# wyhlovecpp/GPT-Image-Edit

Hardware: AMD Instinct MI355X
Metric: edited images/sec, 28-step FLUX-Kontext (VAE encode + 28 x MMDiT + VAE decode) (higher is better)
Workload: dtype bf16; 1 GPU; cfg2_single_512x512_28step; batch_per_gpu=1, global_batch=1, height=512, width=512, S_txt=512, S_tgt=1024, S_cond=1024, seq_len=2560, num_inference_steps=28, blocks=19 double + 38 single, parallelism=dp1

## Files before the change

### gpt_image_edit_amd/csrc/gemm_epilogue.h

```cpp
#pragma once

#include "mxfp8_quant.h"

constexpr int BM = 256;

struct TileRows {
  int ld, wrap, rpb, b0, r0;
  int rf;
  float inv;
  bool big;
  FK_DEV TileRows(const fk_rows& r, int m0, bool flat = false) {
    ld = (int)r.ld;
    if (flat) { rpb = 0x7fffffff; wrap = 0; b0 = 0; r0 = rf = m0; big = true; inv = 0.f; }
    else if (r.rows_per_batch <= 0) { rpb = 0x7fffffff; wrap = 0; b0 = 0; r0 = 0; rf = m0; big = true; inv = 0.f; }
    else {
      rpb = (int)(r.rows_per_batch > 0x7fffffff ? 0x7fffffff : r.rows_per_batch);
      b0 = (unsigned)m0 / (unsigned)rpb;
      r0 = rf = m0 - b0 * rpb;
      wrap = (int)(r.batch_stride - (int64_t)rpb * r.ld);
      big = rpb >= BM;
      inv = 1.0f / (float)rpb;
    }
  }
  FK_DEV int crossed(int ml) const {
    const int r = r0 + ml;
    const int one = r >= rpb ? 1 : 0;
    const int many = (int)(((float)r + 0.5f) * inv);
    return big ? one : many;
  }
  FK_DEV int off(int ml) const { return ml * ld + crossed(ml) * wrap; }
  FK_DEV int64_t first(const fk_rows& r) const {
    return (int64_t)b0 * r.batch_stride + (int64_t)rf * r.ld;
  }
};

template <int N>
FK_DEV float row_ror(float v) {
  return __int_as_float(__builtin_amdgcn_update_dpp(0, __float_as_int(v), 0x120 + N, 0xf, 0xf, false));
}
FK_DEV float row16_sum(float v) {
  v += row_ror<8>(v);
  v += row_ror<4>(v);
  v += row_ror<2>(v);
  v += row_ror<1>(v);
  return v;
}

FK_DEV int xcd_chunk_index() {
  const int nwg = gridDim.x;
  const int q = nwg >> 3, r = nwg & 7;
  const int xcd = blockIdx.x & 7, idx = blockIdx.x >> 3;
  return (xcd < r ? xcd * (q + 1) : r * (q + 1) + (xcd - r) * q) + idx;
}

template <bool M16>
struct FragMap {
  static FK_DEV int row(int lane, int q) { return M16 ? (q & 1) * 16 + (lane & 15) : (lane & 31); }
  static FK_DEV int col(int lane, int q) { return M16 ? (q >> 1) * 16 + (lane >> 4) * 4 : 8 * q + 4 * (lane >> 5); }
};
FK_DEV f32x4_t quad_get(const f32x16_t& v, int q) { return f32x4_t{v[4 * q], v[4 * q + 1], v[4 * q + 2], v[4 * q + 3]}; }
FK_DEV void quad_set(f32x16_t& v, int q, const f32x4_t& c) {
  v[4 * q] = c[0]; v[4 * q + 1] = c[1]; v[4 * q + 2] = c[2]; v[4 * q + 3] = c[3];
}

constexpr int WALK_CT_OFF = 65536;
FK_DEV void lds_barrier() { asm volatile("s_waitcnt lgkmcnt(0)\n\ts_barrier" ::: "memory"); }
template <int EPI, int BN, class C, int HALF = -1, int UB = 8, bool WALK = false>
FK_DEV void store_tile(const f32x16_t (&acc)[C::NF][C::MF], const fk_gemm_args& p, char* smem, int m0, int n0,
                       int wm, int wn, const u32x4_t* other = nullptr, int flat = 0, const u32x2_t (*bias_in)[4] = nullptr) {
  constexpr bool ADD_OTHER = HALF >= 0 && !WALK;
  constexpr int MF0 = HALF > 0 ? C::MF / 2 : 0, MF1 = HALF == 0 ? C::MF / 2 : C::MF;
  constexpr int row0 = HALF > 0 ? BM / 2 : 0;
  int tid = threadIdx.x;
  if constexpr (C::NTHREADS == 256 || WALK) asm volatile("" : "+v"(tid));
  const int lane = tid & 63;
  using FM = FragMap<C::M16>;
  u32x2_t bw[C::NF][4];
#pragma unroll
  for (int nf = 0; nf < C::NF; ++nf)
#pragma unroll
    for (int q = 0; q < 4; ++q) bw[nf][q] = u32x2_t{0u, 0u};
  if constexpr (WALK) {
#pragma unroll
    for (int nf = 0; nf < C::NF; ++nf)
#pragma unroll
      for (int q = 0; q < 4; ++q) bw[nf][q] = bias_in[nf][q];
  } else if constexpr (EPI != FK_EPI_SCALE) {
    if (p.bias) {
#pragma unroll
      for (int nf = 0; nf < C::NF; ++nf)
#pragma unroll
        for (int q = 0; q < 4; ++q) {
          const int n = n0 + C::tile_col(wn, nf) + FM::col(lane, q);
          bw[nf][q] = *(const u32x2_t*)((const bf16_t*)p.bias + min(n, p.N - 4));
        }
    }
  }
  if constexpr (EPI == FK_EPI_F32DBG) {
#pragma unroll
    for (int nf = 0; nf < C::NF; ++nf)
#pragma unroll
      for (int q = 0; q < 4; ++q) {
        const int n = n0 + C::tile_col(wn, nf) + FM::col(lane, q);
        const float b[4] = {bf_lo(bw[nf][q][0]), bf_hi(bw[nf][q][0]), bf_lo(bw[nf][q][1]), bf_hi(bw[nf][q][1])};
#pragma unroll
        for (int mf = MF0; mf < MF1; ++mf) {
          const int m = m0 + C::tile_row(wm, mf) + FM::row(lane, q);
          f32x4_t x = quad_get(acc[nf][mf], q);
          if constexpr (HALF >= 0) {
#pragma unroll
            for (int j = 0; j < 4; ++j) x[j] += __uint_as_float(other[nf * 2 * C::MF + (mf - MF0) * 4 + q][j]);
          }
          if (m < p.M && n < p.N)
            *(f32x4_t*)((float*)p.C + fk_row_offset(p.c, m) + n) = f32x4_t{x[0] + b[0], x[1] + b[1], x[2] + b[2], x[3] + b[3]};
        }
      }
    return;
  }
  if constexpr (WALK) lds_barrier(); else __syncthreads();
  bf16_t* ct = WALK ? (bf16_t*)(smem + WALK_CT_OFF) - row0 * C::CT_LD : (bf16_t*)smem;
#pragma unroll
  for (int nf = 0; nf < C::NF; ++nf) {
#pragma unroll
    for (int q = 0; q < 4; ++q) {
      const int nl = C::tile_col(wn, nf) + FM::col(lane, q);
      const float b[4] = {bf_lo(bw[nf][q][0]), bf_hi(bw[nf][q][0]), bf_lo(bw[nf][q][1]), bf_hi(bw[nf][q][1])};
#pragma unroll
      for (int mf = MF0; mf < MF1; ++mf) {
        float v[4];
#pragma unroll
        for (int j = 0; j < 4; ++j) {
          float x = acc[nf][mf][q * 4 + j];
          if constexpr (ADD_OTHER) x += __uint_as_float(other[nf * 2 * C::MF + (mf - MF0) * 4 + q][j]);
          if constexpr (EPI == FK_EPI_SCALE) v[j] = x * p.alpha;
          else v[j] = x + b[j];
        }
        if constexpr (EPI == FK_EPI_GELU_TANH || EPI == FK_EPI_SILU) {
          round_bf_pair(v[0], v[1]);
          round_bf_pair(v[2], v[3]);
#pragma unroll
          for (int j = 0; j < 4; ++j) v[j] = EPI == FK_EPI_GELU_TANH ? gelu_tanh_f(v[j]) : silu_f(v[j]);
        }
        u32x2_t pk;
        pk[0] = pack_bf2(v[0], v[1]);
        pk[1] = pack_bf2(v[2], v[3]);
        const int ml = C::tile_row(wm, mf) + FM::row(lane, q);
        *(u32x2_t*)(ct + ml * C::CT_LD + nl) = pk;
      }
    }
  }
  if constexpr (WALK) lds_barrier(); else __syncthreads();
  if constexpr (WALK && HALF <= 0) asm volatile("s_waitcnt vmcnt(0)" ::: "memory");
  constexpr int CPR = BN / 8;
  constexpr int ITERS = (HALF >= 0 ? BM / 2 : BM) * CPR / C::NTHREADS;
  constexpr int U = (EPI == FK_EPI_QKV && (ITERS > 8 || HALF >= 0)) ? 4 : UB;
  static_assert(ITERS % U == 0 && C::NTHREADS % CPR == 0, "epilogue batching");
  constexpr bool HAS_RES = EPI == FK_EPI_GATE_RES || EPI == FK_EPI_RES;
  const bool cflat = flat & 2, rflat = flat & 4, gflat = flat & 8;
  const TileRows crow(p.c, m0, cflat);
  bf16_t* const cbase = (bf16_t*)p.C + crow.first(p.c);
  const TileRows rrow = HAS_RES ? TileRows(p.r, m0, rflat) : crow;
  const bf16_t* const rbase = HAS_RES ? (const bf16_t*)p.res + rrow.first(p.r) : nullptr;
  fk_rows gr = {0, 0, 0};
  if constexpr (EPI == FK_EPI_GATE_RES) gr.rows_per_batch = p.gate_rows_per_batch;
  const TileRows grow(gr, m0, gflat);
  const int D = EPI == FK_EPI_QKV ? p.qkv_heads * 128 : 1;
  const int which = EPI == FK_EPI_QKV ? n0 / D : 0;
  const int cc = tid % CPR, ml0 = row0 + tid / CPR;
  constexpr int ML_STEP = C::NTHREADS / CPR;
  const int n = n0 + cc * 8;
  const int nc = min(n, p.N - 8);
  const int mlast = p.M - 1 - m0;

  if (EPI == FK_EPI_QKV && which < 2) {
    const int hn = n - which * D;
    const int head = hn >> 7, dch = hn & 127;
    const u32x4_t ww = *(const u32x4_t*)((const bf16_t*)(which == 0 ? p.wq : p.wk) + dch);
    bf16_t* const dst = (bf16_t*)(which == 0 ? p.q_out : p.k_out);
#pragma unroll
    for (int j0 = 0; j0 < ITERS; j0 += U) {
      u32x4_t y[U];
      f32x4_t t0[U], t1[U];
      int srow[U], bidx[U];
#pragma unroll
      for (int u = 0; u < U; ++u) {
        const int ml = ml0 + ML_STEP * (j0 + u);
        y[u] = *(const u32x4_t*)(ct + ml * C::CT_LD + cc * 8);
        const int mlc = min(ml, mlast);
        const int nb = crow.crossed(mlc);
        bidx[u] = crow.b0 + nb;
        srow[u] = p.qkv_s_offset + crow.r0 + mlc - nb * crow.rpb;
        const float* tp = p.rope_cs + (int64_t)srow[u] * 128 + dch;
        t0[u] = *(const f32x4_t*)tp;
        t1[u] = *(const f32x4_t*)(tp + 4);
      }
#pragma unroll
      for (int u = 0; u < U; ++u) {
        const int ml = ml0 + ML_STEP * (j0 + u);
        float xv[8];
        float ss = 0.f;
#pragma unroll
        for (int e = 0; e < 4; ++e) {
          xv[2 * e] = bf_lo(y[u][e]);
          xv[2 * e + 1] = bf_hi(y[u][e]);
          ss += xv[2 * e] * xv[2 * e] + xv[2 * e + 1] * xv[2 * e + 1];
        }
        ss = row16_sum(ss);
        const float rs = __builtin_amdgcn_rsqf(ss * (1.0f / 128) + 1e-6f);
        const float cs[4] = {t0[u][0], t0[u][2], t1[u][0], t1[u][2]};
        const float sn[4] = {t0[u][1], t0[u][3], t1[u][1], t1[u][3]};
        u32x4_t ow;
#pragma unroll
        for (int e = 0; e < 4; ++e) {
          float re = xv[2 * e] * rs, im = xv[2 * e + 1] * rs;
          round_bf_pair(re, im);
          re *= bf_lo(ww[e]);
          im *= bf_hi(ww[e]);
          round_bf_pair(re, im);
          const float o0 = mul2_add(re, cs[e], -im, sn[e]);
          const float o1 = mul2_add(im, cs[e], re, sn[e]);
          ow[e] = pack_bf2(o0, o1);
        }
        const int hrow = (bidx[u] * p.qkv_heads + head) * p.qkv_s_total + srow[u];
        if (ml <= mlast && n < p.N) *(u32x4_t*)(dst + (int64_t)hrow * 128 + dch) = ow;
      }
    }
    return;
  }

#pragma unroll
  for (int j0 = 0; j0 < ITERS; j0 += U) {
    u32x4_t y[U], rv[U], gv[U];
    int coff[U];
#pragma unroll
    for (int u = 0; u < U; ++u) {
      const int ml = ml0 + ML_STEP * (j0 + u);
      const int mlc = min(ml, mlast);
      y[u] = *(const u32x4_t*)(ct + ml * C::CT_LD + cc * 8);
      coff[u] = crow.off(mlc) + n;
      if constexpr (EPI == FK_EPI_GATE_RES || EPI == FK_EPI_RES) rv[u] = *(const u32x4_t*)(rbase + rrow.off(mlc) + nc);
      if constexpr (EPI == FK_EPI_GATE_RES) {
        const int64_t b = grow.b0 + grow.crossed(mlc);
        gv[u] = *(const u32x4_t*)((const bf16_t*)p.gate + b * p.gate_batch_stride + nc);
      }
    }
#pragma unroll
    for (int u = 0; u < U; ++u) {
      const int ml = ml0 + ML_STEP * (j0 + u);
      u32x4_t o = y[u];
      if constexpr (EPI == FK_EPI_GATE_RES || EPI == FK_EPI_RES) {
#pragma unroll
        for (int e = 0; e < 4; ++e) {
          float y0 = bf_lo(o[e]), y1 = bf_hi(o[e]);
          if constexpr (EPI == FK_EPI_GATE_RES) {
            y0 *= bf_lo(gv[u][e]);
            y1 *= bf_hi(gv[u][e]);
            round_bf_pair(y0, y1);
          }
          o[e] = pack_bf2(bf_lo(rv[u][e]) + y0, bf_hi(rv[u][e]) + y1);
        }
      }
      if (ml <= mlast && n < p.N) *(u32x4_t*)(cbase + coff[u]) = o;
    }
  }
}

template <int EPI, int BN, class C>
FK_DEV void store_tile_mxq(const f32x16_t (&acc)[C::NF][C::MF], const fk_gemm_args& p, uint8_t* __restrict__ q,
                           uint8_t* __restrict__ s, int64_t ldq, int64_t ld_scale, char* smem, int m0, int n0, int wm, int wn) {
  static_assert(EPI == FK_EPI_NONE || EPI == FK_EPI_GELU_TANH, "quantized output: plain and GELU epilogues");
  const int tid = threadIdx.x, lane = tid & 63;
  using FM = FragMap<C::M16>;
  u32x2_t bw[C::NF][4];
#pragma unroll
  for (int nf = 0; nf < C::NF; ++nf)
#pragma unroll
    for (int qd = 0; qd < 4; ++qd) bw[nf][qd] = u32x2_t{0u, 0u};
  if (p.bias) {
#pragma unroll
    for (int nf = 0; nf < C::NF; ++nf)
#pragma unroll
      for (int qd = 0; qd < 4; ++qd) {
        const int n = n0 + C::tile_col(wn, nf) + FM::col(lane, qd);
        bw[nf][qd] = *(const u32x2_t*)((const bf16_t*)p.bias + min(n, p.N - 4));
      }
  }
  __syncthreads();
  bf16_t* ct = (bf16_t*)smem;
#pragma unroll
  for (int nf = 0; nf < C::NF; ++nf) {
#pragma unroll
    for (int qd = 0; qd < 4; ++qd) {
      const int nl = C::tile_col(wn, nf) + FM::col(lane, qd);
      const float b[4] = {bf_lo(bw[nf][qd][0]), bf_hi(bw[nf][qd][0]), bf_lo(bw[nf][qd][1]), bf_hi(bw[nf][qd][1])};
#pragma unroll
      for (int mf = 0; mf < C::MF; ++mf) {
        float v[4];
#pragma unroll
        for (int j = 0; j < 4; ++j) v[j] = acc[nf][mf][qd * 4 + j] + b[j];
        if constexpr (EPI == FK_EPI_GELU_TANH) {
          round_bf_pair(v[0], v[1]);
          round_bf_pair(v[2], v[3]);
#pragma unroll
          for (int j = 0; j < 4; ++j) v[j] = gelu_tanh_f(v[j]);
        }
        u32x2_t pk;
        pk[0] = pack_bf2(v[0], v[1]);
        pk[1] = pack_bf2(v[2], v[3]);
        const int ml = C::tile_row(wm, mf) + FM::row(lane, qd);
        *(u32x2_t*)(ct + ml * C::CT_LD + nl) = pk;
      }
    }
  }
  __syncthreads();
  constexpr int BPR = BN / 32;
  constexpr int ITERS = BM * BPR / C::NTHREADS;
  constexpr int ML_STEP = C::NTHREADS / BPR;
  static_assert(C::NTHREADS % BPR == 0 && (BM * BPR) % C::NTHREADS == 0, "quantized epilogue tiling");
  const int bc = tid % BPR, ml0 = tid / BPR;
  const int mlast = p.M - 1 - m0;
#pragma unroll
  for (int j = 0; j < ITERS; ++j) {
    const int ml = ml0 + ML_STEP * j;
    const u32x4_t* src = (const u32x4_t*)(ct + ml * C::CT_LD + bc * 32);
    uint32_t w[16], out[8];
#pragma unroll
    for (int i = 0; i < 4; ++i) {
      const u32x4_t v = src[i];
      w[4 * i] = v[0]; w[4 * i + 1] = v[1]; w[4 * i + 2] = v[2]; w[4 * i + 3] = v[3];
    }
    const uint32_t sbyte = mx_quant_block(w, out);
    if (ml <= mlast) {
      const int64_t m = (int64_t)m0 + ml;
      u32x4_t* dst = (u32x4_t*)(q + m * ldq + n0 + bc * 32);
      dst[0] = u32x4_t{out[0], out[1], out[2], out[3]};
      dst[1] = u32x4_t{out[4], out[5], out[6], out[7]};
      s[m * ld_scale + (n0 >> 5) + bc] = (uint8_t)sbyte;
    }
  }
}
```

### gpt_image_edit_amd/csrc/gemm_pingpong_bf16.hip

```cpp
#include <stdlib.h>

#include <type_traits>

#include "fk_common.h"

namespace {

#include "gemm_epilogue.h"
#define FK_TM_FN __host__ __device__ __forceinline__
#include "gemm_tile_map.h"
static_assert(TM_MAX_GROUP == FK_MAX_GROUP && TM_BM == BM, "gemm_tile_map.h mirrors fk.h / gemm_epilogue.h");
#ifndef FK_GROUP_M
#define FK_GROUP_M 8
#endif
constexpr int GROUP_M = FK_GROUP_M;
#ifndef FK_RATE_256
#define FK_RATE_256 1.22
#endif


enum { SK_WHOLE = 0, SK_SYM = 1, SK_SYM_UNANNOUNCED = 2 };

struct GroupArgs {
  TileEntry e;
// ... 7 lines not shown
};


#ifdef FK_ENTRY_STAMPS
__device__ unsigned long long* fk_entry_stamp_buf = nullptr;
struct EntryStamps {
  unsigned long long t[5];
  template <int I> FK_DEV void mark() { t[I] = __builtin_amdgcn_s_memtime(); }
  FK_DEV void flush() const {
    if (threadIdx.x == 0 && fk_entry_stamp_buf) {
      unsigned long long* r = fk_entry_stamp_buf + (size_t)blockIdx.x * 8;
      for (int i = 0; i < 5; ++i) r[i] = t[i];
      r[5] = (unsigned long long)__builtin_amdgcn_s_getreg(63492) | ((unsigned long long)__builtin_amdgcn_s_getreg(63508) << 32);
    }
  }
};
#else
struct EntryStamps {
  template <int I> FK_DEV void mark() {}
  FK_DEV void flush() const {}
};
#endif

typedef __attribute__((address_space(3))) void lds_void;
typedef __attribute__((address_space(1))) const void gbl_void;

typedef short s16x4_t __attribute__((ext_vector_type(4)));
FK_DEV s16x4_t lds_tr16(const char* p) {
  return __builtin_amdgcn_ds_read_tr16_b64_v4i16((__attribute__((address_space(3))) s16x4_t*)p);
}

FK_DEV void buffer_lds16(__amdgpu_buffer_rsrc_t rsrc, char* lds_dst, int voffset, int soffset) {
#if defined(__HIP_DEVICE_COMPILE__)
  __builtin_amdgcn_raw_ptr_buffer_load_lds(rsrc, (lds_void*)lds_dst, 16, voffset, soffset, 0, 0);
#else
  (void)rsrc; (void)lds_dst; (void)voffset; (void)soffset;
#endif
}

FK_DEV void buffer_lds16(const BufDesc& d, char* lds_dst, int voffset, int soffset) {
  buffer_lds_opaque<16>(d, lds_addr_of(lds_dst), voffset, soffset);
}

template <int N>
FK_DEV void wait_vmcnt() {
  if constexpr (N == 0) asm volatile("s_waitcnt vmcnt(0)" ::: "memory");
  else if constexpr (N == 2) asm volatile("s_waitcnt vmcnt(2)" ::: "memory");
  else if constexpr (N == 4) asm volatile("s_waitcnt vmcnt(4)" ::: "memory");
  else if constexpr (N == 6) asm volatile("s_waitcnt vmcnt(6)" ::: "memory");
  else if constexpr (N == 8) asm volatile("s_waitcnt vmcnt(8)" ::: "memory");
  else if constexpr (N == 10) asm volatile("s_waitcnt vmcnt(10)" ::: "memory");
  else if constexpr (N == 12) asm volatile("s_waitcnt vmcnt(12)" ::: "memory");
  else if constexpr (N == 7) asm volatile("s_waitcnt vmcnt(7)" ::: "memory");
  else static_assert(N == 0, "add the vmcnt literal");
}


struct Hot {
  TmHot h;
  uint32_t xq, xr, grid;
  int nk;
};
#define FK_PIN_CLASS(h)                                                                                                   \
  "+s"((h).before[0]), "+s"((h).before[1]), "+s"((h).before[2]), "+s"((h).nbm[0]), "+s"((h).nbm[1]), "+s"((h).nbm[2]),       \
      "+s"((h).nbm[3]), "+s"((h).last_mul[0]), "+s"((h).last_mul[1]), "+s"((h).last_mul[2]), "+s"((h).last_mul[3]),          \
      "+s"((h).per_group), "+s"((h).col0), "+s"((h).per_group_mul), "+s"((h).group_m_mul)
#define FK_PIN_HEAD(x) "+s"((x).h.n), "+s"((x).h.group_m), "+s"((x).xq), "+s"((x).xr), "+s"((x).grid), "+s"((x).nk)
FK_DEV Hot load_hot(const GroupArgs& ga) {
  Hot x;
  x.h = tm_hot(ga.e, ga.e.cls[0]);
  x.xq = ga.e.xq; x.xr = ga.e.xr; x.grid = ga.e.grid; x.nk = ga.e.nk;
  asm volatile("" : FK_PIN_HEAD(x), FK_PIN_CLASS(x.h));
  return x;
}
FK_DEV ProbEntry load_prob(const GroupArgs& ga, int pi) {
  ProbEntry q = ga.pe[pi];
  asm volatile("" : "+s"(q.A), "+s"(q.W), "+s"(q.lda), "+s"(q.ldw), "+s"(q.M), "+s"(q.N), "+s"(q.K), "+s"(q.flags));
  return q;
}
template <int BN>
FK_DEV void select_tile(const Hot& x, int t, int& pi, int& m0, int& n0) { tm_tile_hot(x.h, BN, t, pi, m0, n0); }
FK_DEV int xcd_chunk_of(const Hot& x) { return tm_xcd_chunk(x.xq, x.xr, blockIdx.x); }

FK_DEV int behind_requests(int pi) {
  pi = __builtin_amdgcn_readfirstlane(pi);
  asm volatile("" : "+s"(pi) :: "memory");
  return pi;
}

template <int NR>
FK_DEV int64_t tile_a_rows(const GroupArgs& ga, int pi, const ProbEntry& q, int m0, const int (&rl)[NR], int (&off)[NR]) {
#pragma unroll
  for (int i = 0; i < NR; ++i) off[i] = min(rl[i], q.M - 1 - m0) * q.lda;
  int64_t first = (int64_t)m0 * q.lda;
  if (__builtin_expect(!(q.flags & TM_A_FLAT), 0)) {
    const fk_rows& a = ga.p[pi].a;
    const TileRows arow(a, m0);
#pragma unroll
    for (int i = 0; i < NR; ++i) off[i] = arow.off(min(rl[i], q.M - 1 - m0));
    first = arow.first(a);
  }
  return first;
}

FK_DEV void mma16_block(f32x16_t& blk, const bf16x8_t& w0, const bf16x8_t& w1, const bf16x8_t& a0, const bf16x8_t& a1) {
  quad_set(blk, 0, __builtin_amdgcn_mfma_f32_16x16x32_bf16(w0, a0, quad_get(blk, 0), 0, 0, 0));
  quad_set(blk, 2, __builtin_amdgcn_mfma_f32_16x16x32_bf16(w1, a0, quad_get(blk, 2), 0, 0, 0));
  quad_set(blk, 1, __builtin_amdgcn_mfma_f32_16x16x32_bf16(w0, a1, quad_get(blk, 1), 0, 0, 0));
  quad_set(blk, 3, __builtin_amdgcn_mfma_f32_16x16x32_bf16(w1, a1, quad_get(blk, 3), 0, 0, 0));
}



template <int BN, bool M16_ = false>
struct Cfg8 {
  static_assert(BN == 256, "the ping-pong kernel is instantiated for the 256 x 256 tile only");
  static constexpr bool M16 = M16_;
  static constexpr int NTHREADS = 512;
  static constexpr int BK = 64, ROW_BYTES = 128;
  static constexpr int WAVES_M = 2, WAVES_N = 4;
  static constexpr int MF = 4, NF = 2;
  static constexpr int HALF_BYTES = 128 * ROW_BYTES;
  static constexpr int BUF_BYTES = 4 * HALF_BYTES;
  static constexpr int RING_BYTES = 2 * BUF_BYTES;
  static constexpr int CT_LD = BN + 8;
  static constexpr int CT_BYTES = BM * CT_LD * 2;
  static constexpr int SMEM_BYTES = RING_BYTES > CT_BYTES ? RING_BYTES : CT_BYTES;
  static FK_DEV int swz(int row) { return (row >> 1) & 7; }
  static FK_DEV int tile_row(int wm, int mf) { return (mf >> 1) * 128 + wm * 64 + (mf & 1) * 32; }
  static FK_DEV int tile_col(int wn, int nf) { return nf * 128 + wn * 32; }
};

template <int EPI, int BN, int LAY = 0, bool M16 = false, bool SYM = false>
FK_DEV void gemm8_body(const GroupArgs& ga, char* smem, int pi, int m0, int n0, int kt_first, int nk, int sk_slot, int sk_part = 0, EntryStamps* st = nullptr) {
  EntryStamps st_none;
  if (!st) st = &st_none;
  using C = Cfg8<BN, M16>;
  constexpr bool AT = LAY == 2, WT = LAY >= 1;
  const int tid = threadIdx.x;
  const int lane = tid & 63;
  const int wave = __builtin_amdgcn_readfirstlane(tid >> 6);
  const int wm = wave >> 2, wn = wave & 3;
  const ProbEntry q = load_prob(ga, pi);
  const int kbase = kt_first * (C::BK * 2);

  const int lrow = lane >> 3, slot = lane & 7;
  const int prow = lane >> 4, pslot = lane & 15;
  int a_voff[2][2], w_voff[2][2];
  int64_t a_first = m0;
  {
    const int ldw2 = q.ldw * 2, lda2 = q.lda * 2;
    int rls[4], aoff[4] = {0, 0, 0, 0};
#pragma unroll
    for (int i = 0; i < 4; ++i) rls[i] = (i >> 1) * 128 + (wave * 2 + (i & 1)) * 8 + lrow;
    if constexpr (!AT) a_first = tile_a_rows<4>(ga, pi, q, m0, rls, aoff);
#pragma unroll
    for (int h = 0; h < 2; ++h)
#pragma unroll
      for (int j = 0; j < 2; ++j) {
        const int rl = rls[h * 2 + j];
        const int sw = (slot ^ C::swz(rl)) << 4;
        const int kl = (wave * 2 + j) * 4 + prow;
        const int ct = (h * 128 + (((((pslot >> 2) ^ prow) << 2) | (pslot & 3)) << 3)) * 2;
        a_voff[h][j] = AT ? kl * lda2 + ct : aoff[h * 2 + j] * 2 + sw;
        w_voff[h][j] = WT ? kl * ldw2 + ct : min(rl, q.N - 1 - n0) * ldw2 + sw;
      }
  }
  const bf16_t* const a_src = (const bf16_t*)q.A + a_first;
  const bf16_t* const w_src = (const bf16_t*)q.W + (WT ? (int64_t)n0 : (int64_t)n0 * q.ldw);
  const __amdgpu_buffer_rsrc_t rs_a = __builtin_amdgcn_make_buffer_rsrc((void*)a_src, 0, 0x7fffffff, 0x00020000);
  const __amdgpu_buffer_rsrc_t rs_w = __builtin_amdgcn_make_buffer_rsrc((void*)w_src, 0, 0x7fffffff, 0x00020000);
  const BufDesc od_a = make_buf_desc(a_src, 0x7fffffffu);
  const BufDesc od_w = make_buf_desc(w_src, 0x7fffffffu);
  const int kstep_a = AT ? C::BK * q.lda * 2 : C::BK * 2, kstep_w = WT ? C::BK * q.ldw * 2 : C::BK * 2;
  auto dma_half = [&](int which, int buf, int kt) {
    const int ktc = min(kt, nk - 1);
    char* dst = smem + buf * C::BUF_BYTES + which * C::HALF_BYTES + wave * 2048;
    if (which < 2) {
      const int koff = (AT ? 0 : kbase) + ktc * kstep_a;
      if constexpr (AT || WT) {
        buffer_lds16(od_a, dst, a_voff[which][0], koff);
        buffer_lds16(od_a, dst + 1024, a_voff[which][1], koff);
      } else {
        buffer_lds16(rs_a, dst, a_voff[which][0], koff);
        buffer_lds16(rs_a, dst + 1024, a_voff[which][1], koff);
      }
    } else {
      const int koff = (WT ? 0 : kbase) + ktc * kstep_w;
      if constexpr (AT || WT) {
        buffer_lds16(od_w, dst, w_voff[which - 2][0], koff);
        buffer_lds16(od_w, dst + 1024, w_voff[which - 2][1], koff);
      } else {
        buffer_lds16(rs_w, dst, w_voff[which - 2][0], koff);
        buffer_lds16(rs_w, dst + 1024, w_voff[which - 2][1], koff);
      }
    }
  };

  dma_half(2, 0, 0);
  st->mark<1>();
  dma_half(0, 0, 0);
  dma_half(3, 0, 0);
  dma_half(1, 0, 0);
  dma_half(2, 1, 1);
  dma_half(0, 1, 1);
  dma_half(3, 1, 1);
  const fk_gemm_args& p = ga.p[behind_requests(pi)];
  unsigned sk_ann = 0;
  if constexpr (SYM) {
    if (ga.sk_mode != SK_WHOLE && wave == 0) {
      unsigned r = 0;
      if (lane == 0)
        r = __hip_atomic_fetch_add((__attribute__((address_space(1))) unsigned*)(ga.sk_ctl + 2 * (size_t)sk_slot), 1u, __ATOMIC_RELAXED,
                                   __HIP_MEMORY_SCOPE_AGENT);
      sk_ann = __builtin_amdgcn_readfirstlane(r);
    }
  }

  constexpr int NKS = M16 ? 2 : 4;
  constexpr int ASUB = M16 ? 4 : 2;
  constexpr int WSUB = M16 ? 2 : 1;
  constexpr int SUB_BYTES = (M16 ? 16 : 32) * C::ROW_BYTES;
  const int frow = M16 ? (lane & 15) : (lane & 31), fhalf = M16 ? (lane >> 4) : (lane >> 5), fsw = C::swz(frow);
  int koffs[NKS];
#pragma unroll
  for (int kk = 0; kk < NKS; ++kk) koffs[kk] = ((kk * (M16 ? 4 : 2) + fhalf) ^ fsw) << 4;
  const int a_rd = (wm * 64 + frow) * C::ROW_BYTES;
  const int w_rd = (wn * 32 + frow) * C::ROW_BYTES;

  f32x16_t acc[C::NF][C::MF];
#pragma unroll
  for (int i = 0; i < C::NF; ++i)
#pragma unroll
    for (int j = 0; j < C::MF; ++j)
#pragma unroll
      for (int r = 0; r < 16; ++r) acc[i][j][r] = 0.f;

  bf16x8_t af[ASUB][NKS], wf[2][WSUB][NKS];
  const int tj = (lane & 15) >> 2;
  const int t_lo = M16 ? (8 * (lane >> 4) + tj) * 256 + (lane & 3) * 8
                       : (8 * (lane >> 5) + tj) * 256 + ((lane >> 4) & 1) * 32 + (lane & 3) * 8;
  auto trfrag = [&](const char* half, int kk, int df) {
    const char* vp = M16 ? half + kk * 8192 + (((df >> 1) ^ tj) << 6) + (df & 1) * 32 + t_lo
                         : half + kk * 4096 + ((df ^ tj) << 6) + t_lo;
    const s16x4_t lo = lds_tr16(vp);
    const s16x4_t hi = lds_tr16(vp + 4 * 256);
    bf16x8_t f;
    f[0] = lo[0]; f[1] = lo[1]; f[2] = lo[2]; f[3] = lo[3];
    f[4] = hi[0]; f[5] = hi[1]; f[6] = hi[2]; f[7] = hi[3];
    return f;
  };
  auto read_a = [&](int buf, int h) {
    const char* b = smem + buf * C::BUF_BYTES + h * C::HALF_BYTES;
#pragma unroll
    for (int sub = 0; sub < ASUB; ++sub)
#pragma unroll
      for (int kk = 0; kk < NKS; ++kk) {
        if constexpr (AT) af[sub][kk] = trfrag(b, kk, wm * ASUB + sub);
        else af[sub][kk] = *(const bf16x8_t*)(b + a_rd + sub * SUB_BYTES + koffs[kk]);
      }
  };
  auto read_w = [&](int buf, int j) {
    const char* b = smem + buf * C::BUF_BYTES + (2 + j) * C::HALF_BYTES;
#pragma unroll
    for (int sub = 0; sub < WSUB; ++sub)
#pragma unroll
      for (int kk = 0; kk < NKS; ++kk) {
        if constexpr (WT) wf[j][sub][kk] = trfrag(b, kk, wn * WSUB + sub);
        else wf[j][sub][kk] = *(const bf16x8_t*)(b + w_rd + sub * SUB_BYTES + koffs[kk]);
      }
  };
  auto mma = [&](int i, int j) {
#pragma unroll
    for (int kk = 0; kk < NKS; ++kk)
#pragma unroll
      for (int sub = 0; sub < 2; ++sub) {
        if constexpr (M16) mma16_block(acc[j][2 * i + sub], wf[j][0][kk], wf[j][1][kk], af[2 * sub][kk], af[2 * sub + 1][kk]);
        else acc[j][2 * i + sub] = __builtin_amdgcn_mfma_f32_32x32x16_bf16(wf[j][0][kk], af[sub][kk], acc[j][2 * i + sub], 0, 0, 0);
      }
  };
  auto phase_sync_mma = [&](int i, int j) {
    wait_vmcnt<10>();
    __builtin_amdgcn_sched_barrier(0);
    __builtin_amdgcn_s_barrier();
    asm volatile("s_waitcnt lgkmcnt(0)" ::: "memory");
    __builtin_amdgcn_sched_barrier(0);
    __builtin_amdgcn_s_setprio(1);
    mma(i, j);
    __builtin_amdgcn_s_setprio(0);
    __builtin_amdgcn_sched_barrier(0);
    __builtin_amdgcn_s_barrier();
    __builtin_amdgcn_sched_barrier(0);
  };

  wait_vmcnt<10>();
  __builtin_amdgcn_sched_barrier(0);
  __builtin_amdgcn_s_barrier();
  __builtin_amdgcn_sched_barrier(0);
  read_w(0, 0);
  if (wm == 1) __builtin_amdgcn_s_barrier();
  __builtin_amdgcn_sched_barrier(0);
  st->mark<2>();

  auto tile_body = [&](auto bc, int kt) {
    constexpr int b = decltype(bc)::value;
    read_a(b, 0);            dma_half(1, b ^ 1, kt + 1);  phase_sync_mma(0, 0);
    read_w(b, 1);            dma_half(2, b, kt + 2);      phase_sync_mma(0, 1);
    read_a(b, 1);            dma_half(0, b, kt + 2);      phase_sync_mma(1, 0);
    read_w(b ^ 1, 0);        dma_half(3, b, kt + 2);      phase_sync_mma(1, 1);
  };
  for (int kt = 0; kt < nk; kt += 2) {
    tile_body(std::integral_constant<int, 0>{}, kt);
    if (kt + 1 < nk) tile_body(std::integral_constant<int, 1>{}, kt + 1);
  }
  st->mark<3>();
  if (wm == 0) __builtin_amdgcn_s_barrier();
  asm volatile("s_waitcnt vmcnt(0)" ::: "memory");

  if (SYM || sk_slot >= 0) {
    typedef __attribute__((address_space(1))) unsigned gu32;
    gu32* const ctl = (gu32*)(ga.sk_ctl + 2 * (size_t)sk_slot);
    const __amdgpu_buffer_rsrc_t rs_p = __builtin_amdgcn_make_buffer_rsrc(
        (void*)(ga.sk_partials + (size_t)sk_slot * (BM * BN)), 0, BM * BN * 4, 0x00020000);
    const bool announced = SYM && ga.sk_mode != SK_WHOLE;
    __syncthreads();
    if (tid == 0) {
      const unsigned t = __hip_atomic_fetch_add(ctl, announced ? 1u : 2u, __ATOMIC_RELAXED, __HIP_MEMORY_SCOPE_AGENT);
      unsigned role;
      if (!announced) role = (t & 2u) ? 1u : 0u;
      else {
        const bool blind = ga.sk_mode == SK_SYM_UNANNOUNCED;
        if ((t & 3u) == 3u) role = (blind || (sk_ann & 3u) == 2u) ? 1u : 2u;
        else role = ((t & 3u) == 2u && !blind) ? 2u : 0u;
      }
      ((volatile unsigned*)smem)[0] = t;
      ((volatile unsigned*)smem)[1] = role;
    }
    __syncthreads();
    const unsigned ticket = __builtin_amdgcn_readfirstlane(((volatile unsigned*)smem)[0]);
    const unsigned role = __builtin_amdgcn_readfirstlane(((volatile unsigned*)smem)[1]);
    const unsigned target = (ticket & ~3u) + 4u;
    auto wait_flag = [&]() {
      if (tid == 0) {
        int spins = 0;
        while (__hip_atomic_load(ctl + 1, __ATOMIC_RELAXED, __HIP_MEMORY_SCOPE_AGENT) != target && spins < (1 << 22)) {
          __builtin_amdgcn_s_sleep(8);
          ++spins;
        }
        __builtin_amdgcn_fence(__ATOMIC_ACQUIRE, "agent");
      }
      __syncthreads();
    };
    auto publish = [&](unsigned step) {
      asm volatile("s_waitcnt vmcnt(0)" ::: "memory");
      __syncthreads();
      if (tid == 0) __hip_atomic_fetch_add(ctl + 1, step, __ATOMIC_RELAXED, __HIP_MEMORY_SCOPE_AGENT);
    };
    constexpr int NV = C::NF * C::MF * 4, NH = NV / 2;
    auto piece_acc = [&](int r) -> f32x16_t& { return acc[(r % NH) / 8][2 * (r / NH) + (r / 4) % 2]; };
    auto store_piece = [&](int r, int at) {
      const f32x16_t& a = piece_acc(r);
      const int q = r & 3;
      const u32x4_t v = {__float_as_uint(a[4 * q]), __float_as_uint(a[4 * q + 1]), __float_as_uint(a[4 * q + 2]),
                         __float_as_uint(a[4 * q + 3])};
      __builtin_amdgcn_raw_buffer_store_b128(v, rs_p, tid * 16, at * (C::NTHREADS * 16),  16);
    };
    auto finish_half = [&](auto keep_c) {
      constexpr int keep = decltype(keep_c)::value;
      u32x4_t other[NH];
#pragma unroll
      for (int r = 0; r < NH; ++r)
        other[r] = __builtin_amdgcn_raw_buffer_load_b128(rs_p, tid * 16, (keep * NH + r) * (C::NTHREADS * 16),  16);
      store_tile<EPI, BN, C, keep>(acc, p, smem, m0, n0, wm, wn, other, q.flags);
    };
    if constexpr (SYM) {
      if (role == 2u) {
        if (sk_part == 0) {
#pragma unroll
          for (int r = 0; r < NH; ++r) store_piece(NH + r, NH + r);
        } else {
#pragma unroll
          for (int r = 0; r < NH; ++r) store_piece(r, r);
        }
        publish(2u);
        wait_flag();
        if (sk_part == 0) finish_half(std::integral_constant<int, 0>{});
        else finish_half(std::integral_constant<int, 1>{});
        return;
      }
    }
    if (role == 0u) {
#pragma unroll
      for (int r = 0; r < NV; ++r) store_piece(r, r);
      publish(4u);
      return;
    }
    wait_flag();
    if constexpr (SYM) {
      finish_half(std::integral_constant<int, 0>{});
      finish_half(std::integral_constant<int, 1>{});
      return;
    }
#pragma unroll
    for (int r0 = 0; r0 < NV; r0 += 4) {
      u32x4_t v[4];
#pragma unroll
      for (int u = 0; u < 4; ++u)
        v[u] = __builtin_amdgcn_raw_buffer_load_b128(rs_p, tid * 16, (r0 + u) * (C::NTHREADS * 16),  16);
#pragma unroll
      for (int u = 0; u < 4; ++u) {
        f32x16_t& a = piece_acc(r0 + u);
        const int q = u;
#pragma unroll
        for (int j = 0; j < 4; ++j) a[4 * q + j] += __uint_as_float(v[u][j]);
      }
      __builtin_amdgcn_sched_barrier(0);
    }
  }
  store_tile<EPI, BN, C>(acc, p, smem, m0, n0, wm, wn, nullptr, q.flags);
}

template <int EPI, int BN, bool SPLITK, int LAY = 0, bool M16 = false>
__global__ __launch_bounds__(512, 2) void gemm8_kernel(const GroupArgs ga) {
  extern __shared__ __attribute__((aligned(16))) char smem[];
  EntryStamps st;
  st.mark<0>();
  int pi, m0, n0;
  const Hot x = load_hot(ga);
  const int t = xcd_chunk_of(x);
  const int nk_all = x.nk;
  if constexpr (SPLITK) {
    select_tile<BN>(x, t >> 1, pi, m0, n0);
    gemm8_body<EPI, BN, LAY, M16, true>(ga, smem, pi, m0, n0, (t & 1) * (nk_all >> 1), nk_all >> 1, t >> 1, t & 1, &st);
  } else {
    select_tile<BN>(x, t, pi, m0, n0);
    gemm8_body<EPI, BN, LAY, M16>(ga, smem, pi, m0, n0, 0, nk_all, -1, 0, &st);
  }
  st.mark<4>();
  st.flush();
}

struct Cfg10 {
  static constexpr bool M16 = true;
  static constexpr int NTHREADS = 256;
  static constexpr int BK = 64, ROW_BYTES = 128;
  static constexpr int MF = 4, NF = 4;
  static constexpr int HALF_BYTES = 128 * ROW_BYTES;
  static constexpr int BUF_BYTES = 4 * HALF_BYTES;
  static constexpr int RING_BYTES = 2 * BUF_BYTES;
  static constexpr int CT_LD = 256 + 8;
  static constexpr int CT_BYTES = BM * CT_LD * 2;
  static constexpr int SMEM_BYTES = RING_BYTES > CT_BYTES ? RING_BYTES : CT_BYTES;
  static FK_DEV int tile_row(int wm, int mf) { return wm * 128 + mf * 32; }
  static FK_DEV int tile_col(int wn, int nf) { return wn * 128 + nf * 32; }
};
typedef int i32x8_t __attribute__((ext_vector_type(8)));
typedef int i32x4_t __attribute__((ext_vector_type(4)));

#define G10_V4(a) "v" #a "0", "v" #a "1", "v" #a "2", "v" #a "3"
#define G10_V10(a) "v" #a "0", "v" #a "1", "v" #a "2", "v" #a "3", "v" #a "4", "v" #a "5", "v" #a "6", "v" #a "7", "v" #a "8", "v" #a "9"
#define G10_CLOBBER_V64_255 \
  "v64", "v65", "v66", "v67", "v68", "v69", G10_V10(7), G10_V10(8), G10_V10(9), G10_V10(10), G10_V10(11), G10_V10(12), G10_V10(13), \
  G10_V10(14), G10_V10(15), G10_V10(16), G10_V10(17), G10_V10(18), G10_V10(19), G10_V10(20), G10_V10(21), G10_V10(22), G10_V10(23), \
  G10_V10(24), "v250", "v251", "v252", "v253", "v254", "v255"
#define G10_OPERANDS \
      : "={a[0:15]}"(acc[0][0]), "={a[16:31]}"(acc[0][1]), "={a[32:47]}"(acc[0][2]), "={a[48:63]}"(acc[0][3]), \
        "={a[64:79]}"(acc[1][0]), "={a[80:95]}"(acc[1][1]), "={a[96:111]}"(acc[1][2]), "={a[112:127]}"(acc[1][3]), \
        "={a[128:143]}"(acc[2][0]), "={a[144:159]}"(acc[2][1]), "={a[160:175]}"(acc[2][2]), "={a[176:191]}"(acc[2][3]), \
        "={a[192:207]}"(acc[3][0]), "={a[208:223]}"(acc[3][1]), "={a[224:239]}"(acc[3][2]), "={a[240:255]}"(acc[3][3]) \
      : "{v[16:23]}"(a_voff), "{v[24:31]}"(w_voff), "{v[32:39]}"(rd), "{v[40:43]}"(wr), "{s[40:43]}"(od_a.w), "{s[44:47]}"(od_w.w), \
        "{s48}"(k0), "{s49}"(nks), "{s50}"(kmax) \
      : "memory", "scc", "s52", "s53", "s54", G10_CLOBBER_V64_255

#define G10_OPERANDS_X \
      : "={a[0:15]}"(acc[0][0]), "={a[16:31]}"(acc[0][1]), "={a[32:47]}"(acc[0][2]), "={a[48:63]}"(acc[0][3]), \
        "={a[64:79]}"(acc[1][0]), "={a[80:95]}"(acc[1][1]), "={a[96:111]}"(acc[1][2]), "={a[112:127]}"(acc[1][3]), \
        "={a[128:143]}"(acc[2][0]), "={a[144:159]}"(acc[2][1]), "={a[160:175]}"(acc[2][2]), "={a[176:191]}"(acc[2][3]), \
        "={a[192:207]}"(acc[3][0]), "={a[208:223]}"(acc[3][1]), "={a[224:239]}"(acc[3][2]), "={a[240:255]}"(acc[3][3]), "={s[56:57]}"(t0), "={s[58:59]}"(t1), "={s[60:61]}"(ta) \
      : "{v[16:23]}"(a_voff), "{v[24:31]}"(w_voff), "{v[32:39]}"(rd), "{v[40:43]}"(wr), "{s[40:43]}"(od_a.w), "{s[44:47]}"(od_w.w), \
        "{s48}"(k0), "{s49}"(nks), "{s50}"(kmax) \
      : "memory", "scc", "s52", "s53", "s54", G10_CLOBBER_V64_255

template <int EPI, int V = 0>
FK_DEV void gemm10_body(const GroupArgs& ga, char* smem, int pi, int m0, int n0, int kt_first, int nk) {
  using C = Cfg10;
#ifdef FK_G10_EXPERIMENTS
  const unsigned long long g10_real0 = __builtin_amdgcn_s_memrealtime(), g10_cyc0 = __builtin_amdgcn_s_memtime();
#endif
  int tid = threadIdx.x;
  asm volatile("" : "+v"(tid));
  const int lane = tid & 63;
  const int wave = __builtin_amdgcn_readfirstlane(tid >> 6);
  const int wm = wave >> 1, wn = wave & 1;
  const ProbEntry q = load_prob(ga, pi);
  const int lrow = lane >> 3, chunk = lane & 7;
  i32x8_t a_voff, w_voff;
  int64_t a_first;
  {
    const int ldw2 = q.ldw * 2;
    int rls[8], aoff[8];
#pragma unroll
    for (int i = 0; i < 8; ++i) rls[i] = wave * 64 + i * 8 + lrow;
    a_first = tile_a_rows<8>(ga, pi, q, m0, rls, aoff);
#pragma unroll
    for (int i = 0; i < 8; ++i) {
      a_voff[i] = aoff[i] * 2 + chunk * 16;
      w_voff[i] = min(rls[i], q.N - 1 - n0) * ldw2 + chunk * 16;
    }
  }
  const BufDesc od_a = make_buf_desc((const bf16_t*)q.A + a_first, 0x7fffffffu);
  const BufDesc od_w = make_buf_desc((const bf16_t*)q.W + (int64_t)n0 * q.ldw, 0x7fffffffu);
  const int base = (int)lds_addr_of(smem);
  i32x8_t rd;
  i32x4_t wr;
  {
    const int frow = lane & 15, fhalf = lane >> 4, fsw = (frow >> 1) & 7;
#pragma unroll
    for (int buf = 0; buf < 2; ++buf)
#pragma unroll
      for (int kk = 0; kk < 2; ++kk) {
        const int ko = ((kk * 4 + fhalf) ^ fsw) << 4;
        rd[2 * buf + kk] = base + buf * C::BUF_BYTES + wm * C::HALF_BYTES + frow * C::ROW_BYTES + ko;
        rd[4 + 2 * buf + kk] = base + buf * C::BUF_BYTES + (2 + wn) * C::HALF_BYTES + frow * C::ROW_BYTES + ko;
      }
#pragma unroll
    for (int buf = 0; buf < 2; ++buf)
#pragma unroll
      for (int par = 0; par < 2; ++par)
        wr[2 * buf + par] = base + buf * C::BUF_BYTES + (wave >> 1) * C::HALF_BYTES + (wave & 1) * 8192 + lrow * C::ROW_BYTES +
                            ((chunk ^ ((par * 4 + (lrow >> 1)) & 7)) << 4);
  }
  const int k0 = __builtin_amdgcn_readfirstlane(kt_first * (C::BK * 2));
  const int nks = __builtin_amdgcn_readfirstlane(nk);
  const int kmax = k0 + (nks - 1) * (C::BK * 2);

  f32x16_t acc[C::NF][C::MF];
  if constexpr (V == 0) {
    asm volatile(
#include "gemm10_loop.inc"
        G10_OPERANDS);
  }
#ifdef FK_G10_EXPERIMENTS
  unsigned long long t0 = 0, t1 = 0, ta = 0;
  (void)t0; (void)t1; (void)ta;
  if constexpr (V == 1) { asm volatile(
#include "gemm10_loop_x1.inc"
        G10_OPERANDS_X); }
  else if constexpr (V == 2) { asm volatile(
#include "gemm10_loop_x2.inc"
        G10_OPERANDS_X); }
  else if constexpr (V == 3) { asm volatile(
#include "gemm10_loop_x3.inc"
        G10_OPERANDS_X); }
  else if constexpr (V == 4) { asm volatile(
#include "gemm10_loop_x4.inc"
        G10_OPERANDS_X); }
  else if constexpr (V == 5) { asm volatile(
#include "gemm10_loop_x5.inc"
        G10_OPERANDS_X); }
  else if constexpr (V == 6) { asm volatile(
#include "gemm10_loop_x6.inc"
        G10_OPERANDS_X); }
  else if constexpr (V == 7) { asm volatile(
#include "gemm10_loop_x7.inc"
        G10_OPERANDS_X); }
  else if constexpr (V == 8) { asm volatile(
#include "gemm10_loop_x8.inc"
        G10_OPERANDS_X); }
  else if constexpr (V == 9) { asm volatile(
#include "gemm10_loop_x9.inc"
        G10_OPERANDS_X); }
  else if constexpr (V == 10) { asm volatile(
#include "gemm10_loop_x10.inc"
        G10_OPERANDS_X); }
  else if constexpr (V == 11) { asm volatile(
#include "gemm10_loop_x11.inc"
        G10_OPERANDS_X); }
  else if constexpr (V == 12) { asm volatile(
#include "gemm10_loop_x12.inc"
        G10_OPERANDS_X); }
  else if constexpr (V == 13) { asm volatile(
#include "gemm10_loop_x13.inc"
        G10_OPERANDS_X); }
  else if constexpr (V == 14) { asm volatile(
#include "gemm10_loop_x14.inc"
        G10_OPERANDS_X); }
  else if constexpr (V == 15) { asm volatile(
#include "gemm10_loop_x15.inc"
        G10_OPERANDS_X); }
  else if constexpr (V == 16) { asm volatile(
#include "gemm10_loop_x16.inc"
        G10_OPERANDS_X); }
  else if constexpr (V == 17) { asm volatile(
#include "gemm10_loop_x17.inc"
        G10_OPERANDS_X); }
  else if constexpr (V == 18) { asm volatile(
#include "gemm10_loop_x18.inc"
        G10_OPERANDS_X); }
  else if constexpr (V == 19) { asm volatile(
#include "gemm10_loop_x19.inc"
        G10_OPERANDS_X); }
  else if constexpr (V == 20) { asm volatile(
#include "gemm10_loop_x20.inc"
        G10_OPERANDS_X); }
#endif
  const fk_gemm_args& p = ga.p[behind_requests(pi)];
  store_tile<EPI, 256, C>(acc, p, smem, m0, n0, wm, wn, nullptr, q.flags);
#ifdef FK_G10_EXPERIMENTS
  if constexpr (V > 0) {
    if (tid == 0) {
      unsigned long long* rec = (unsigned long long*)((bf16_t*)p.C + (int64_t)p.M * p.c.ld) + (size_t)blockIdx.x * 8;
      rec[0] = (unsigned long long)__builtin_amdgcn_s_getreg(63492) | ((unsigned long long)__builtin_amdgcn_s_getreg(63508) << 32);
      rec[1] = g10_real0; rec[2] = __builtin_amdgcn_s_memrealtime();
      rec[3] = g10_cyc0; rec[4] = t0; rec[5] = t1; rec[6] = __builtin_amdgcn_s_memtime();
      rec[7] = ta;
    }
  }
#endif
}

template <int EPI, int V = 0, bool PERSIST = false>
__global__ __launch_bounds__(256, 1) void gemm10_kernel(const GroupArgs ga) {
  extern __shared__ __attribute__((aligned(16))) char smem[];
  const Hot x = load_hot(ga);
  const int nk = x.nk;
  if constexpr (PERSIST) {
    const int total = ga.e.cls[0].before[FK_MAX_GROUP];
    for (int t = xcd_chunk_of(x); t < total; t += (int)x.grid) {
      int pi, m0, n0;
      select_tile<256>(x, t, pi, m0, n0);
      gemm10_body<EPI, V>(ga, smem, pi, m0, n0, 0, nk);
      asm volatile("s_waitcnt lgkmcnt(0)\n\ts_barrier" ::: "memory");
    }
  } else {
    int pi, m0, n0;
    select_tile<256>(x, xcd_chunk_of(x), pi, m0, n0);
    gemm10_body<EPI, V>(ga, smem, pi, m0, n0, 0, nk);
  }
}

template <int EPI, int BN, bool M16 = false>
__global__ __launch_bounds__(512, 2) void gemm8_streamk_kernel(const GroupArgs ga) {
  extern __shared__ __attribute__((aligned(16))) char smem[];
  const Hot x = load_hot(ga);
  const int pos = xcd_chunk_of(x);
  const unsigned G = x.grid, nk = (unsigned)x.nk;
  const unsigned U = (unsigned)ga.e.cls[0].before[FK_MAX_GROUP] * nk, qU = U / G, rU = U - qU * G;
  auto cut = [&](unsigned j) __attribute__((always_inline)) {
    unsigned c = qU * j + (rU * j) / G;
    const unsigned r = c % nk;
    if (r != 0 && r < (unsigned)ga.sk_min_part) c -= r;
    else if (r != 0 && nk - r < (unsigned)ga.sk_min_part) c += nk - r;
    return (int)c;
  };
  const int u = cut(pos);
  int u_end = cut(pos + 1);
  while (u < u_end) {
    const int t = (unsigned)(u_end - 1) / nk;
    const int k1 = u_end - t * (int)nk, k0 = max(u - t * (int)nk, 0);
    u_end -= k1 - k0;
    int pi, m0, n0;
    select_tile<BN>(x, t, pi, m0, n0);
    const bool part = k0 > 0 || k1 < (int)nk;
    gemm8_body<EPI, BN, 0, M16>(ga, smem, pi, m0, n0, k0, k1 - k0, part ? (k1 < (int)nk ? pos + 1 : pos) : -1);
    __syncthreads();
  }
}

template <int BN>
int count_tiles(GroupArgs& ga, const fk_gemm_args* probs, int n, int grid = 0, bool split = false) {
  int32_t Ms[FK_MAX_GROUP];
  for (int i = 0; i < n; ++i) Ms[i] = probs[i].M;
  const int total = tm_fill_class(ga.e.cls[0], Ms, n, (probs[0].N + BN - 1) / BN, 0, ga.e.group_m);
  if (total >= 0) tm_fill_grid(ga.e, (uint32_t)(grid ? grid : split ? 2 * total : total));
  return total;
}

template <int EPI, int BN, bool SPLITK, int LAY = 0, bool M16 = false>
int launch8(GroupArgs& ga, const fk_gemm_args* probs, int n, hipStream_t stream) {
  const int total = count_tiles<BN>(ga, probs, n, 0, SPLITK);
  if (total < 0) return FK_E2BIG_STRIDES;
  auto kern = gemm8_kernel<EPI, BN, SPLITK, LAY, M16>;
  FK_ENSURE_MAX_LDS(kern, Cfg8<BN>::SMEM_BYTES, "fk_gemm_bf16 (256 x 256 tile, 8 waves ping-pong)");
  hipLaunchKernelGGL(kern, dim3(SPLITK ? 2 * total : total), dim3(512), Cfg8<BN>::SMEM_BYTES, stream, ga);
  FK_CHECK_LAUNCH("fk_gemm_bf16 (256 x 256 tile, 8 waves ping-pong)");
  return FK_OK;
}

template <int EPI, int BN, bool M16 = false>
int launch8_streamk(GroupArgs& ga, const fk_gemm_args* probs, int n, int grid, hipStream_t stream) {
// ... 963 lines not shown
```

Baseline: 1.112 images/s.

## Draw stream-K ticket early and preload epilogue operands before partner wait

In the symmetric stream-K GEMM path, the atomic ticket is now drawn a couple of k-tiles before the main loop ends, so its latency overlaps the remaining MMA work. The symmetric finish preloads bias, residual and flat gate values into registers before publishing and waiting on the partner CTA, which hides those global loads behind the wait. Some __syncthreads are replaced with lighter LDS barriers. In exchange it uses more registers during the epilogue and moves the ticket ordering earlier in the loop, which could affect occupancy and the correctness of the role assignment.

```diff
diff --git a/gpt_image_edit_amd/csrc/gemm_epilogue.h b/gpt_image_edit_amd/csrc/gemm_epilogue.h
--- a/gpt_image_edit_amd/csrc/gemm_epilogue.h
+++ b/gpt_image_edit_amd/csrc/gemm_epilogue.h
@@ -65,9 +65,67 @@
 
 constexpr int WALK_CT_OFF = 65536;
 FK_DEV void lds_barrier() { asm volatile("s_waitcnt lgkmcnt(0)\n\ts_barrier" ::: "memory"); }
-template <int EPI, int BN, class C, int HALF = -1, int UB = 8, bool WALK = false>
+
+template <int EPI, int BN, class C, int HALF>
+struct EpiRows {
+  static constexpr bool HAS_RES = EPI == FK_EPI_GATE_RES || EPI == FK_EPI_RES;
+  static constexpr int CPR = BN / 8;
+  static constexpr int ITERS = (HALF >= 0 ? BM / 2 : BM) * CPR / C::NTHREADS;
+  static constexpr int ML_STEP = C::NTHREADS / CPR;
+  static constexpr int row0 = HALF > 0 ? BM / 2 : 0;
+  TileRows rrow;
+  const bf16_t* rbase;
+  int ml0, nc, mlast;
+  FK_DEV EpiRows(const fk_gemm_args& p, int m0, int n0, int tid, int flat) : rrow(p.r, m0, flat & 4) {
+    rbase = (const bf16_t*)p.res + rrow.first(p.r);
+    ml0 = row0 + tid / CPR;
+    nc = min(n0 + (tid % CPR) * 8, p.N - 8);
+    mlast = p.M - 1 - m0;
+  }
+  FK_DEV u32x4_t res(int j) const { return *(const u32x4_t*)(rbase + rrow.off(min(ml0 + ML_STEP * j, mlast)) + nc); }
+};
+template <int EPI, int BN, class C, int HALF>
+struct EpiPre {
+  using R = EpiRows<EPI, BN, C, HALF>;
+  static_assert(!R::HAS_RES || R::ITERS <= 8, "one batch of the output loop");
+  u32x2_t bw[C::NF][4];
+  u32x4_t rv[R::HAS_RES ? R::ITERS : 1], g0;
+};
+template <int EPI, int BN, class C, int HALF>
+FK_DEV void epi_preload(EpiPre<EPI, BN, C, HALF>& pre, const fk_gemm_args& p, int m0, int n0, int wn, int flat) {
+  using R = EpiRows<EPI, BN, C, HALF>;
+  const int tid = threadIdx.x, lane = tid & 63;
+#pragma unroll
+  for (int nf = 0; nf < C::NF; ++nf)
+#pragma unroll
+    for (int q = 0; q < 4; ++q) pre.bw[nf][q] = u32x2_t{0u, 0u};
+  if constexpr (EPI != FK_EPI_SCALE) {
+    if (p.bias) {
+#pragma unroll
+      for (int nf = 0; nf < C::NF; ++nf)
+#pragma unroll
+        for (int q = 0; q < 4; ++q) {
+          const int n = n0 + C::tile_col(wn, nf) + FragMap<C::M16>::col(lane, q);
+          pre.bw[nf][q] = *(const u32x2_t*)((const bf16_t*)p.bias + min(n, p.N - 4));
+        }
+    }
+  }
+  pre.g0 = u32x4_t{0u, 0u, 0u, 0u};
+  if constexpr (R::HAS_RES) {
+    const R er(p, m0, n0, tid, flat);
+#pragma unroll
+    for (int j = 0; j < R::ITERS; ++j) pre.rv[j] = er.res(j);
+    if constexpr (EPI == FK_EPI_GATE_RES) {
+      if (flat & 8) pre.g0 = *(const u32x4_t*)((const bf16_t*)p.gate + er.nc);
+    }
+  }
+}
+
+template <int EPI, int BN, class C, int HALF = -1, int UB = 8, bool WALK = false, bool PRE = false>
 FK_DEV void store_tile(const f32x16_t (&acc)[C::NF][C::MF], const fk_gemm_args& p, char* smem, int m0, int n0,
-                       int wm, int wn, const u32x4_t* other = nullptr, int flat = 0, const u32x2_t (*bias_in)[4] = nullptr) {
+                       int wm, int wn, const u32x4_t* other = nullptr, int flat = 0, const u32x2_t (*bias_in)[4] = nullptr,
+                       const EpiPre<EPI, BN, C, HALF>* pre = nullptr) {
+  static_assert(!(PRE && WALK), "the tile walk hands in its bias quads only");
   constexpr bool ADD_OTHER = HALF >= 0 && !WALK;
   constexpr int MF0 = HALF > 0 ? C::MF / 2 : 0, MF1 = HALF == 0 ? C::MF / 2 : C::MF;
   constexpr int row0 = HALF > 0 ? BM / 2 : 0;
@@ -85,6 +143,11 @@
     for (int nf = 0; nf < C::NF; ++nf)
 #pragma unroll
       for (int q = 0; q < 4; ++q) bw[nf][q] = bias_in[nf][q];
+  } else if constexpr (PRE) {
+#pragma unroll
+    for (int nf = 0; nf < C::NF; ++nf)
+#pragma unroll
+      for (int q = 0; q < 4; ++q) bw[nf][q] = pre->bw[nf][q];
   } else if constexpr (EPI != FK_EPI_SCALE) {
     if (p.bias) {
 #pragma unroll
@@ -238,10 +301,21 @@
       const int mlc = min(ml, mlast);
       y[u] = *(const u32x4_t*)(ct + ml * C::CT_LD + cc * 8);
       coff[u] = crow.off(mlc) + n;
-      if constexpr (EPI == FK_EPI_GATE_RES || EPI == FK_EPI_RES) rv[u] = *(const u32x4_t*)(rbase + rrow.off(mlc) + nc);
-      if constexpr (EPI == FK_EPI_GATE_RES) {
-        const int64_t b = grow.b0 + grow.crossed(mlc);
-        gv[u] = *(const u32x4_t*)((const bf16_t*)p.gate + b * p.gate_batch_stride + nc);
+      if constexpr (PRE) {
+        if constexpr (HAS_RES) rv[u] = pre->rv[j0 + u];
+        if constexpr (EPI == FK_EPI_GATE_RES) {
+          gv[u] = pre->g0;
+          if (!gflat) {
+            const int64_t b = grow.b0 + grow.crossed(mlc);
+            gv[u] = *(const u32x4_t*)((const bf16_t*)p.gate + b * p.gate_batch_stride + nc);
+          }
+        }
+      } else {
+        if constexpr (EPI == FK_EPI_GATE_RES || EPI == FK_EPI_RES) rv[u] = *(const u32x4_t*)(rbase + rrow.off(mlc) + nc);
+        if constexpr (EPI == FK_EPI_GATE_RES) {
+          const int64_t b = grow.b0 + grow.crossed(mlc);
+          gv[u] = *(const u32x4_t*)((const bf16_t*)p.gate + b * p.gate_batch_stride + nc);
+        }
       }
     }
 #pragma unroll
diff --git a/gpt_image_edit_amd/csrc/gemm_pingpong_bf16.hip b/gpt_image_edit_amd/csrc/gemm_pingpong_bf16.hip
--- a/gpt_image_edit_amd/csrc/gemm_pingpong_bf16.hip
+++ b/gpt_image_edit_amd/csrc/gemm_pingpong_bf16.hip
@@ -333,9 +333,27 @@
   __builtin_amdgcn_sched_barrier(0);
   st->mark<2>();
 
+  constexpr int SK_DRAW_AHEAD = 2;
+  static_assert(SK_DRAW_AHEAD >= 1 && SK_DRAW_AHEAD <= 2, "a ticket drawn earlier would stand in front of requests that are read");
+  const bool sk_meet = SYM || sk_slot >= 0;
+  const bool sk_announced = SYM && ga.sk_mode != SK_WHOLE;
+  const int kt_draw = SYM && wave == 0 ? max(nk - SK_DRAW_AHEAD, 0) : -1;
+  unsigned sk_ticket = 0;
+  unsigned sk_lane0 = 0;
+  asm volatile("" : "+v"(sk_lane0));
+  auto draw_ticket = [&](int kt) {
+    if constexpr (!SYM) return;
+    if (kt == kt_draw && lane == 0) {
+      typedef __attribute__((address_space(1))) char gchar;
+      gchar* const word = (gchar*)(ga.sk_ctl + 2 * (size_t)sk_slot);
+      sk_ticket = __hip_atomic_fetch_add((__attribute__((address_space(1))) unsigned*)(word + sk_lane0), sk_announced ? 1u : 2u,
+                                         __ATOMIC_RELAXED, __HIP_MEMORY_SCOPE_AGENT);
+    }
+  };
+
   auto tile_body = [&](auto bc, int kt) {
     constexpr int b = decltype(bc)::value;
-    read_a(b, 0);            dma_half(1, b ^ 1, kt + 1);  phase_sync_mma(0, 0);
+    read_a(b, 0);            dma_half(1, b ^ 1, kt + 1);  draw_ticket(kt);  phase_sync_mma(0, 0);
     read_w(b, 1);            dma_half(2, b, kt + 2);      phase_sync_mma(0, 1);
     read_a(b, 1);            dma_half(0, b, kt + 2);      phase_sync_mma(1, 0);
     read_w(b ^ 1, 0);        dma_half(3, b, kt + 2);      phase_sync_mma(1, 1);
@@ -348,15 +366,17 @@
   if (wm == 0) __builtin_amdgcn_s_barrier();
   asm volatile("s_waitcnt vmcnt(0)" ::: "memory");
 
-  if (SYM || sk_slot >= 0) {
+  if (sk_meet) {
     typedef __attribute__((address_space(1))) unsigned gu32;
     gu32* const ctl = (gu32*)(ga.sk_ctl + 2 * (size_t)sk_slot);
     const __amdgpu_buffer_rsrc_t rs_p = __builtin_amdgcn_make_buffer_rsrc(
         (void*)(ga.sk_partials + (size_t)sk_slot * (BM * BN)), 0, BM * BN * 4, 0x00020000);
-    const bool announced = SYM && ga.sk_mode != SK_WHOLE;
-    __syncthreads();
+    const bool announced = sk_announced;
+    typedef __attribute__((address_space(3))) volatile u32x2_t lds_u32x2;
+    lds_u32x2* const sk_words = (lds_u32x2*)smem;
     if (tid == 0) {
-      const unsigned t = __hip_atomic_fetch_add(ctl, announced ? 1u : 2u, __ATOMIC_RELAXED, __HIP_MEMORY_SCOPE_AGENT);
+      unsigned t = sk_ticket;
+      if constexpr (!SYM) t = __hip_atomic_fetch_add(ctl, 2u, __ATOMIC_RELAXED, __HIP_MEMORY_SCOPE_AGENT);
       unsigned role;
       if (!announced) role = (t & 2u) ? 1u : 0u;
       else {
@@ -364,12 +384,12 @@
         if ((t & 3u) == 3u) role = (blind || (sk_ann & 3u) == 2u) ? 1u : 2u;
         else role = ((t & 3u) == 2u && !blind) ? 2u : 0u;
       }
-      ((volatile unsigned*)smem)[0] = t;
-      ((volatile unsigned*)smem)[1] = role;
-    }
-    __syncthreads();
-    const unsigned ticket = __builtin_amdgcn_readfirstlane(((volatile unsigned*)smem)[0]);
-    const unsigned role = __builtin_amdgcn_readfirstlane(((volatile unsigned*)smem)[1]);
+      *sk_words = u32x2_t{t, role};
+    }
+    lds_barrier();
+    const u32x2_t sk_tr = *sk_words;
+    const unsigned ticket = __builtin_amdgcn_readfirstlane(sk_tr[0]);
+    const unsigned role = __builtin_amdgcn_readfirstlane(sk_tr[1]);
     const unsigned target = (ticket & ~3u) + 4u;
     auto wait_flag = [&]() {
       if (tid == 0) {
@@ -380,7 +400,7 @@
         }
         __builtin_amdgcn_fence(__ATOMIC_ACQUIRE, "agent");
       }
-      __syncthreads();
+      lds_barrier();
     };
     auto publish = [&](unsigned step) {
       asm volatile("s_waitcnt vmcnt(0)" ::: "memory");
@@ -396,27 +416,39 @@
                          __float_as_uint(a[4 * q + 3])};
       __builtin_amdgcn_raw_buffer_store_b128(v, rs_p, tid * 16, at * (C::NTHREADS * 16),  16);
     };
+    auto load_other = [&](int keep, u32x4_t (&other)[NH]) {
+#pragma unroll
+      for (int r = 0; r < NH; ++r)
+        other[r] = __builtin_amdgcn_raw_buffer_load_b128(rs_p, tid * 16, (keep * NH + r) * (C::NTHREADS * 16),  16);
+    };
     auto finish_half = [&](auto keep_c) {
       constexpr int keep = decltype(keep_c)::value;
       u32x4_t other[NH];
-#pragma unroll
-      for (int r = 0; r < NH; ++r)
-        other[r] = __builtin_amdgcn_raw_buffer_load_b128(rs_p, tid * 16, (keep * NH + r) * (C::NTHREADS * 16),  16);
+      load_other(keep, other);
       store_tile<EPI, BN, C, keep>(acc, p, smem, m0, n0, wm, wn, other, q.flags);
+    };
+    auto symmetric = [&](auto keep_c) {
+      constexpr int keep = decltype(keep_c)::value;
+#pragma unroll
+      for (int r = 0; r < NH; ++r) store_piece((1 - keep) * NH + r, (1 - keep) * NH + r);
+      if constexpr (EPI == FK_EPI_QKV || EPI == FK_EPI_F32DBG) {
+        publish(2u);
+        wait_flag();
+        finish_half(keep_c);
+      } else {
+        EpiPre<EPI, BN, C, keep> pre;
+        epi_preload(pre, p, m0, n0, wn, q.flags);
+        publish(2u);
+        wait_flag();
+        u32x4_t other[NH];
+        load_other(keep, other);
+        store_tile<EPI, BN, C, keep, 8, false, true>(acc, p, smem, m0, n0, wm, wn, other, q.flags, nullptr, &pre);
+      }
     };
     if constexpr (SYM) {
       if (role == 2u) {
-        if (sk_part == 0) {
-#pragma unroll
-          for (int r = 0; r < NH; ++r) store_piece(NH + r, NH + r);
-        } else {
-#pragma unroll
-          for (int r = 0; r < NH; ++r) store_piece(r, r);
-        }
-        publish(2u);
-        wait_flag();
-        if (sk_part == 0) finish_half(std::integral_constant<int, 0>{});
-        else finish_half(std::integral_constant<int, 1>{});
+        if (sk_part == 0) symmetric(std::integral_constant<int, 0>{});
+        else symmetric(std::integral_constant<int, 1>{});
         return;
       }
     }
```

Result: no change. 1.106 images/s (-0.5%).
